# ROBOT-WSC/RGC-SLAM

Hardware: AMD Instinct MI355X
Metric: registered scans/sec (16-beam -> 1M-pt map) (higher is better)
Workload: dtype f32 points and neighbour search, f64 covariances and solve

## Files before the change

rgc-slam_amd/csrc/rgc_kernels.hip:

```cpp
#include "rgc_kernels.h"
#include "rgc_nn.h"
#include "rgc_lm.h"
#include "rgc_cov.h"
#include "rgc_terms.h"
#include <hip/hip_ext.h>

#include <limits.h>
#include <stddef.h>

#include <type_traits>

namespace rgck {

constexpr int WAVE = 64;

__device__ __forceinline__ int voxel_coord1(float x, double res) { return (int)floor((double)x / res - 0.5); }

__device__ __forceinline__ int wave_min(int v) {
#pragma unroll
  for (int o = 32; o > 0; o >>= 1) v = min(v, __shfl_xor(v, o));
  return v;
}
__device__ __forceinline__ int wave_max(int v) {
#pragma unroll
// ... 1504 lines not shown
    if (!kFinal) return true;
    defer(~i, (double)thr_up < 3.0 * (R + 1) * (R + 1) * g.res * g.res ? thr_up : INFINITY, 5);
    return false;
  }
  if (!decided) {
    defer(i, thr_up, 6);
    return false;
  }
  const int idx_k = swap ? index_of(a_k) : 0;
  const int m_lo = -(sub & 1), m_hi = -(sub >> 1);
  auto pick4 = [](int mlo, int mhi, int a0, int a1, int a2, int a3) {
    const int x = a0 ^ ((a0 ^ a1) & mlo), y = a2 ^ ((a2 ^ a3) & mlo);
    return x ^ ((x ^ y) & mhi);
  };
  int idx[KC];
  auto positions = [&](auto full_tag) {
    constexpr bool kFull = decltype(full_tag)::value;
#pragma unroll
    for (int t = 0; t < KC / S; t++) {
      const int key = pick4(m_lo, m_hi, all.a[S * t], all.a[S * t + 1], all.a[S * t + 2], all.a[S * t + 3]);
      const int j = S * t + sub;
      all.a[t] = (swap && j == k - 1) ? idx_k : ((kFull || j < k) ? index_of(key) : INT_MAX);
    }
    if (!df.split_sums) {
#pragma unroll
      for (int t = 0; t < KC / S; t++) {
        idx[S * t + 0] = quad_perm_i<0x00>(all.a[t]);
        idx[S * t + 1] = quad_perm_i<0x55>(all.a[t]);
        idx[S * t + 2] = quad_perm_i<0xAA>(all.a[t]);
        idx[S * t + 3] = quad_perm_i<0xFF>(all.a[t]);
      }
      sort_positions<KC>(idx);
      sp_normal_of<KC, kFull>(P, idx, px, py, pz, k, i, nx, ny, nz);
      return;
    }
    double S6[6] = {0, 0, 0, 0, 0, 0}, m3[3] = {0, 0, 0};
    const double qx = (double)px, qy = (double)py, qz = (double)pz;
#pragma unroll
    for (int t = 0; t < KC / S; t++) {
      const bool use = kFull || S * t + sub < k;
      const float4 cp = P[use ? all.a[t] : 0];
      const double dx = use ? (double)cp.x - qx : 0.0, dy = use ? (double)cp.y - qy : 0.0, dz = use ? (double)cp.z - qz : 0.0;
      m3[0] += dx; m3[1] += dy; m3[2] += dz;
      S6[0] = fma(dx, dx, S6[0]); S6[1] = fma(dx, dy, S6[1]); S6[2] = fma(dx, dz, S6[2]);
      S6[3] = fma(dy, dy, S6[3]); S6[4] = fma(dy, dz, S6[4]); S6[5] = fma(dz, dz, S6[5]);
    }
#pragma unroll
    for (int a = 0; a < 3; a++) m3[a] = quad_sum_f64(m3[a]);
#pragma unroll
    for (int a = 0; a < 6; a++) S6[a] = quad_sum_f64(S6[a]);
    normal_from_moments(S6, m3[0], m3[1], m3[2], k, i, nx, ny, nz);
  };
  if (kExact || k == KC) positions(std::true_type{});
  else positions(std::false_type{});
  return false;
}

template <bool kTarget> struct SpConfig {
  static constexpr int KB = kTarget ? 11 : 12;
  static constexpr int R = 1;
  static constexpr bool kClip = !kTarget;
  static constexpr int T = kTarget ? KNN_T : WAVE;
};

#if defined(RGC_LAB) || defined(RGC_LAB_BLK)
#define RGC_LAB_BLOCKS 1
__device__ long long g_lab_blk[4 * 16384];
void lab_blocks(long long* out) {
  (void)hipDeviceSynchronize();
  (void)hipMemcpyFromSymbol(out, HIP_SYMBOL(g_lab_blk), sizeof(g_lab_blk));
}
#endif
#ifdef RGC_LAB
__device__ long long g_lab_wave[2 * 8192];
void lab_wave_ts(long long* out, hipStream_t s) {
  (void)hipStreamSynchronize(s);
  (void)hipMemcpyFromSymbol(out, HIP_SYMBOL(g_lab_wave), sizeof(g_lab_wave));
}
#endif
constexpr int kSeedT = 128;
template <bool kTarget, bool kSeeded> struct SpLaunch : SpConfig<kTarget> {
  static constexpr int T = kSeeded ? kSeedT : SpConfig<kTarget>::T;
};
struct CoopRows {
  int pref[WAVE + 1];
  int rowa[WAVE];
  int nb[32];
};

template <int KC, int R, bool kExact>
__global__ void __launch_bounds__(WAVE)
k_knn_sp_wide(const float4* __restrict__ P, const int* __restrict__ start, Grid g, int n, int k, Deferred df, double* __restrict__ nx,
              double* __restrict__ ny, double* __restrict__ nz) {
  extern __shared__ int slist_wide[];
  if (df.guard && *df.guard) return;
  const int t = (int)blockIdx.x * WAVE + (int)threadIdx.x;
  const int i = t >> 2;
  if (i < n) knn_point_split<KC, SpConfig<false>::KB, R, WAVE, kExact>(P, start, g, n, k, i, t & 3, slist_wide + threadIdx.x, df, nx, ny, nz);
}

__device__ __forceinline__ int wave_sum_i(int v) {
#pragma unroll
  for (int o = 32; o > 0; o >>= 1) v += __shfl_xor(v, o);
  return v;
}
__device__ __forceinline__ int wave_min_i(int v) { return wave_min(v); }



__device__ __forceinline__ int coop_locate(const CoopRows* sh, int j) {
  int rr = 0;
#pragma unroll
  for (int step = 32; step > 0; step >>= 1) {
    const int probe = rr + step;
    if (sh->pref[probe] <= j) rr = probe;
  }
  return sh->rowa[rr] + (j - sh->pref[rr]);
}

template <typename F>
__device__ __forceinline__ void coop_for_each_candidate(const Grid& g, const int c[3], int r, const int* __restrict__ start,
                                                        CoopRows* sh, int lane, F&& f) {
  const int z0 = max(c[2] - r, 0), z1 = min(c[2] + r, g.dim[2] - 1);
  const int y0 = max(c[1] - r, 0), y1 = min(c[1] + r, g.dim[1] - 1);
  const int x0 = max(c[0] - r, 0), x1 = min(c[0] + r, g.dim[0] - 1);
  if (x0 > x1 || y0 > y1 || z0 > z1) return;
  const int ny = y1 - y0 + 1, nrows = ny * (z1 - z0 + 1);
  for (int rb = 0; rb < nrows; rb += WAVE) {
    const int t = rb + lane;
    int a = 0, b = 0;
    if (t < nrows) {
      const int y = y0 + t % ny, z = z0 + t / ny;
      a = start[cell_index(g, x0, y, z)];
      b = start[cell_index(g, x1, y, z) + 1];
    }
    const int len = b - a;
    int inc = len;
#pragma unroll
    for (int o = 1; o < WAVE; o <<= 1) {
      const int u = __shfl_up(inc, o);
      if (lane >= o) inc += u;
    }
    const int total = __shfl(inc, WAVE - 1);
    wave_lds_fence();
    sh->pref[lane] = inc - len;
    sh->rowa[lane] = a;
    if (lane == 0) sh->pref[WAVE] = INT_MAX;
    wave_lds_fence();
    for (int jb = 0; jb < total; jb += 2 * WAVE) {
      const int j0 = jb + lane, j1 = jb + WAVE + lane;
      const bool v0 = j0 < total, v1 = j1 < total;
      const int s0 = v0 ? coop_locate(sh, j0) : 0;
      const int s1 = v1 ? coop_locate(sh, j1) : 0;
      f(s0, v0, s1, v1);
    }
  }
}

template <int KW>
__device__ __forceinline__ unsigned coop_kth(const float4* __restrict__ P, const int* __restrict__ start, const Grid& g, const int c[3], int r,
                                             CoopRows* sh, int lane, float px, float py, float pz, int k, bool& overflow) {
  TopK<KW> top;
  top.init();
  coop_for_each_candidate(g, c, r, start, sh, lane, [&](int s0, bool v0, int s1, bool v1) {
    const float4 c0 = P[s0], c1 = P[s1];
    const float x0 = v0 ? dist2(px, py, pz, c0) : INFINITY;
    const float x1 = v1 ? dist2(px, py, pz, c1) : INFINITY;
    if (top.improves(x0)) top.insert(x0);
    if (top.improves(x1)) top.insert(x1);
  });
  unsigned T = 0;
  for (int bit = 30; bit >= 0; bit--) {
    const unsigned cand = T | (1u << bit);
    if (cand > 0x7F800000u) continue;
    int cnt_lt = 0;
#pragma unroll
    for (int j = 0; j < KW; j++) cnt_lt += __popcll(__ballot(top.a[j] < (int)cand));
    if (cnt_lt < k) T = cand;
  }
  overflow = __any(top.a[KW - 1] < (int)T);
  return T;
}

struct GenOut { double* c6; int method; int n; };
template <int KC>
__device__ __forceinline__ void cov6_of(const float4* __restrict__ P, const int (&idx)[KC], int k, int i, const GenOut& go);

template <int KC, bool kTarget, bool kGeneral = false, bool kLean = false>
__device__ __forceinline__ void coop_one(const float4* __restrict__ P, const int* __restrict__ start, const Grid& g, int k, const Deferred& df,
                                         double* __restrict__ nx, double* __restrict__ ny, double* __restrict__ nz, CoopRows* sh, int lane,
                                         int e, int enc, float thr, const GenOut& go = GenOut{nullptr, 0, 0}) {
  {
#ifdef RGC_LAB
    const long long lab_t0 = wall_clock64();
    int lab_rounds = 0;
#endif
    const int i = enc < 0 ? ~enc : enc;
    int r = enc < 0 ? 1 : 0;
    const float4 pq = P[i];
    const float px = pq.x, py = pq.y, pz = pq.z;
    const int c[3] = {cell_coord(px, g) - g.minc[0], cell_coord(py, g) - g.minc[1], cell_coord(pz, g) - g.minc[2]};
    const double q[3] = {(double)px, (double)py, (double)pz};
    const int rmax = max(max(max(c[0], g.dim[0] - 1 - c[0]), max(c[1], g.dim[1] - 1 - c[1])), max(c[2], g.dim[2] - 1 - c[2]));
    for (;;) {
      int rn;
      if (thr < INFINITY) {
        const double need = sqrt((double)thr) * (1.0 + 1e-5);
        rn = r + 1;
        while (rn < rmax) {
          const double b = cube_bound(g, c, q, rn);
          if (b == 1.0e300 || b > need) break;
          rn++;
        }
      } else {
        rn = r + max(1, (r + 1) / 2);
      }
      r = min(rn, rmax);
      bool overflow;
#ifdef RGC_LAB
      lab_rounds++;
#endif
      unsigned T = coop_kth<4>(P, start, g, c, r, sh, lane, px, py, pz, k, overflow);
      if (overflow) T = coop_kth<KC>(P, start, g, c, r, sh, lane, px, py, pz, k, overflow);
      thr = (T >= 0x7F800000u) ? INFINITY : __uint_as_float(T);
      if (r >= rmax) break;
      if (thr < INFINITY) {
        const double bound = cube_bound(g, c, q, r);
        if (bound == 1.0e300) break;
        if (bound > 0.0 && (double)thr < bound * bound * (1.0 - 1e-5)) break;
      }
    }
    int m = 0;
    int tie_o = INT_MAX, tie_s = -1;
    auto take = [&](int s, bool valid, const float4& cp) {
      const float x = valid ? dist2(px, py, pz, cp) : INFINITY;
      const unsigned long long mask = __ballot(x < thr);
      if (x < thr) {
        const int pos = m + __popcll(mask & ((1ull << lane) - 1ull));
        if (pos < k) sh->nb[pos] = s;
      }
      m += __popcll(mask);
      const int o = __float_as_int(cp.w);
      if (x == thr && o < tie_o) { tie_o = o; tie_s = s; }
    };
    coop_for_each_candidate(g, c, r, start, sh, lane, [&](int s0, bool v0, int s1, bool v1) {
      const float4 c0 = P[s0], c1 = P[s1];
      take(s0, v0, c0);
      take(s1, v1, c1);
    });
    int last_o = -1;
    while (m < k) {
      int best_o = wave_min_i(tie_o);
      if (best_o == INT_MAX) break;
      if (tie_o == best_o) sh->nb[m] = tie_s;
      m++;
      last_o = best_o;
      if (m >= k) break;
      tie_o = INT_MAX;
      tie_s = -1;
      coop_for_each_candidate(g, c, r, start, sh, lane, [&](int s0, bool v0, int s1, bool v1) {
        const float4 c0 = P[s0], c1 = P[s1];
        const int o0 = __float_as_int(c0.w), o1 = __float_as_int(c1.w);
        if (v0 && dist2(px, py, pz, c0) == thr && o0 > last_o && o0 < tie_o) { tie_o = o0; tie_s = s0; }
        if (v1 && dist2(px, py, pz, c1) == thr && o1 > last_o && o1 < tie_o) { tie_o = o1; tie_s = s1; }
      });
    }
    wave_lds_fence();
    {
      const int mine = lane < k ? sh->nb[lane] : INT_MAX;
      int rank = 0;
      for (int j = 0; j < k; j++) rank += sh->nb[j] < mine;
      wave_lds_fence();
      if (lane < k) sh->nb[rank] = mine;
      wave_lds_fence();
    }
    if constexpr (kLean) {
      static_assert(!kGeneral && KC <= 32, "coordinates of up to 32 neighbours in the rows' LDS");
      if (lane < k) {
        const float4 cp = P[sh->nb[lane]];
        sh->pref[lane] = __float_as_int(cp.x); sh->pref[32 + lane] = __float_as_int(cp.y); sh->rowa[lane] = __float_as_int(cp.z);
      }
      wave_lds_fence();
      if (lane == 0) {
        double S[6] = {0, 0, 0, 0, 0, 0};
        const double qx = (double)px, qy = (double)py, qz = (double)pz;
        double mx = 0, my = 0, mz = 0;
#pragma unroll 1
        for (int j = 0; j < k; j++) {
          const double dx = (double)__int_as_float(sh->pref[j]) - qx, dy = (double)__int_as_float(sh->pref[32 + j]) - qy, dz = (double)__int_as_float(sh->rowa[j]) - qz;
          mx += dx; my += dy; mz += dz;
          S[0] = fma(dx, dx, S[0]); S[1] = fma(dx, dy, S[1]); S[2] = fma(dx, dz, S[2]);
          S[3] = fma(dy, dy, S[3]); S[4] = fma(dy, dz, S[4]); S[5] = fma(dz, dz, S[5]);
        }
        normal_from_moments(S, mx, my, mz, k, i, nx, ny, nz);
        if (kTarget && df.seed) df.seed[__float_as_int(pq.w)] = thr;
      }
    } else if (lane == 0) {
      int idx[KC];
#pragma unroll
      for (int j = 0; j < KC; j++) idx[j] = j < k ? sh->nb[j] : 0;
      if constexpr (kGeneral) {
        cov6_of<KC>(P, idx, k, i, go);
      } else {
        if (k == KC) sp_normal_of<KC, true>(P, idx, px, py, pz, k, i, nx, ny, nz);
        else sp_normal_of<KC, false>(P, idx, px, py, pz, k, i, nx, ny, nz);
      }
      if (kTarget && df.seed) df.seed[__float_as_int(pq.w)] = thr;
#ifdef RGC_LAB
      if (!kTarget && e < 8192) { g_lab_wave[2 * e] = lab_t0 | ((long long)r << 56) | ((long long)lab_rounds << 48); g_lab_wave[2 * e + 1] = wall_clock64(); }
#endif
    }
    wave_lds_fence();
  }
}

template <int KC, bool kTarget>
__device__ __forceinline__ void coop_run(const float4* __restrict__ P, const int* __restrict__ start, const Grid& g, int k, const Deferred& df,
                                         double* __restrict__ nx, double* __restrict__ ny, double* __restrict__ nz, CoopRows* sh, int lane,
                                         int wave, int nwaves) {
  const int cnt = *df.cnt;
  for (int e = wave; e < cnt; e += nwaves) {
    const int enc = __builtin_amdgcn_readfirstlane(df.idx[e]);
    const float thr = __int_as_float(__builtin_amdgcn_readfirstlane(__float_as_int(df.thr[e])));
    coop_one<KC, kTarget>(P, start, g, k, df, nx, ny, nz, sh, lane, e, enc, thr);
  }
}
template <int KC, bool kTarget = false>
__device__ __forceinline__ void coop_stream(const float4* __restrict__ P, const int* __restrict__ start, const Grid& g, int k, const Deferred& df,
                            double* __restrict__ nx, double* __restrict__ ny, double* __restrict__ nz, CoopRows* sh, int lane, int wave, int nwaves,
                            int bulk_blocks, int nslots) {
  for (int e = wave;; e += nwaves) {
    if (e >= nslots) return;
    unsigned long long v;
    for (;;) {
      v = __hip_atomic_load(&df.slots[e], __ATOMIC_RELAXED, __HIP_MEMORY_SCOPE_AGENT);
      if (v != kSlotEmpty) break;
      __builtin_amdgcn_s_sleep(20);
    }
    if constexpr (kTarget) {
      const int enc0 = (int)(unsigned)v;
      const unsigned long long left = v == kSlotEnd ? kSlotEmpty : (kSlotResolvedTag | (unsigned long long)(unsigned)(enc0 < 0 ? ~enc0 : enc0));
      if (lane == 0) __hip_atomic_store(&df.slots[e], left, __ATOMIC_RELAXED, __HIP_MEMORY_SCOPE_AGENT);
    } else {
      if (lane == 0) __hip_atomic_store(&df.slots[e], kSlotEmpty, __ATOMIC_RELAXED, __HIP_MEMORY_SCOPE_AGENT);
    }
    if (v == kSlotEnd) return;
    const int enc = __builtin_amdgcn_readfirstlane((int)(unsigned)v);
    const float thr = __int_as_float(__builtin_amdgcn_readfirstlane((int)(unsigned)(v >> 32)));
    coop_one<KC, kTarget, false, kTarget>(P, start, g, k, df, nx, ny, nz, sh, lane, e, enc, thr);
  }
}
__device__ __forceinline__ void coop_count_out(const Deferred& df, int bulk_blocks, int nwaves, int nslots, int* flag) {
  __syncthreads();
  if (threadIdx.x == 0) *flag = __hip_atomic_fetch_add(df.done, 1, __ATOMIC_RELAXED, __HIP_MEMORY_SCOPE_AGENT) == bulk_blocks - 1;
  __syncthreads();
  if (*flag) {
    const int cnt = __hip_atomic_load(df.cnt, __ATOMIC_RELAXED, __HIP_MEMORY_SCOPE_AGENT);
    for (int j = (int)threadIdx.x; j < nwaves; j += (int)blockDim.x)
      if (cnt + j < nslots) __hip_atomic_store(&df.slots[cnt + j], kSlotEnd, __ATOMIC_RELAXED, __HIP_MEMORY_SCOPE_AGENT);
  }
}
struct VoxOut {
  double* vox;
  int* vox_cell;
  const int* cell_voxel;
};
__device__ __forceinline__ void voxel_block_from_search(const float4* __restrict__ P, const int* __restrict__ start, const Grid& g, int n, int i,
                                                        const double (&nrm)[3], const VoxOut& vo, int* lds);
template <int KC, bool kTarget>
__global__ void __launch_bounds__(WAVE)
k_knn_coop(const float4* __restrict__ P, const int* __restrict__ start, Grid g, int k, Deferred df, double* __restrict__ nx,
           double* __restrict__ ny, double* __restrict__ nz) {
  __shared__ CoopRows shm[1];
  wave_prio(!kTarget);
  if (df.guard && *df.guard) return;
  coop_run<KC, kTarget>(P, start, g, k, df, nx, ny, nz, &shm[0], (int)threadIdx.x, (int)blockIdx.x, (int)gridDim.x);
}

template <int KC, bool kTarget, bool kExact, bool kSeeded, bool kVox>
__device__ __forceinline__ void knn_sp_body(const float4* __restrict__ P, const int* __restrict__ start, const Grid& g, int n, int k, const Deferred& df,
                                            double* __restrict__ nx, double* __restrict__ ny, double* __restrict__ nz, const VoxOut& vo) {
  extern __shared__ __align__(16) int slist_sp[];
  using Cfg = SpLaunch<kTarget, kSeeded>;
  static_assert(!kSeeded || (kTarget && kExact), "seeds: the map's search at k == KC");
  wave_prio(!kTarget);
  if (df.guard && *df.guard) return;
  constexpr int kXcdRun = kXcdRunQueries / Cfg::T;
  int b = (int)blockIdx.x, slot = b >> 3;
  const int x = b & 7;
  if constexpr (!kTarget) {
    if (df.coop_blocks > 0 && b >= (int)gridDim.x - df.coop_blocks) {
      const int bulk = (int)gridDim.x - df.coop_blocks;
      coop_stream<KC>(P, start, g, k, df, nx, ny, nz, reinterpret_cast<CoopRows*>(slist_sp) + (threadIdx.x / WAVE), (int)threadIdx.x & (WAVE - 1),
                      (b - bulk) * (Cfg::T / WAVE) + (int)threadIdx.x / WAVE, df.coop_blocks * (Cfg::T / WAVE), bulk, n);
      return;
    }
    const int t = b * Cfg::T + (int)threadIdx.x;
    const int i = t >> 2;
#ifdef RGC_LAB
    const long long lab_t0 = wall_clock64();
#endif
    if (i < n && knn_point_split<KC, Cfg::KB, Cfg::R, Cfg::T, kExact, false>(P, start, g, n, k, i, t & 3, slist_sp + threadIdx.x, df, nx, ny, nz))
      knn_point_split<KC, Cfg::KB, 2, Cfg::T, kExact, true>(P, start, g, n, k, i, t & 3, slist_sp + threadIdx.x, df, nx, ny, nz);
#ifdef RGC_LAB
    if (threadIdx.x == 0 && b < 8192) { g_lab_wave[2 * b] = lab_t0; g_lab_wave[2 * b + 1] = wall_clock64(); }
#endif
    if (df.coop_blocks > 0) coop_count_out(df, (int)gridDim.x - df.coop_blocks, df.coop_blocks * (Cfg::T / WAVE), n, slist_sp);
    return;
  }
  if constexpr (kVox) {
    if (df.coop_blocks > 0 && b >= (int)gridDim.x - df.coop_blocks) {
      const int bulk = (int)gridDim.x - df.coop_blocks;
      coop_stream<KC, true>(P, start, g, k, df, nx, ny, nz, reinterpret_cast<CoopRows*>(slist_sp) + (threadIdx.x / WAVE), (int)threadIdx.x & (WAVE - 1),
                            (b - bulk) * (Cfg::T / WAVE) + (int)threadIdx.x / WAVE, df.coop_blocks * (Cfg::T / WAVE), bulk, n);
      return;
    }
  }
  bool cached = false;
  if constexpr (kSeeded && RGC_KNN_CACHE != 0) {
    if (df.cache.nbr) {
      const bool redo = cache_redo(df.cache);
      if (b < df.cache_nb) {
        if (redo) return;
        Deferred dfb = df;
        dfb.cache.nbr = nullptr;
        const int l = b % kTodoLists, per = df.cache_nb / kTodoLists;
        const int cnt = min(df.cache.todo_cnt[l], df.cache.todo_cap);
        for (int e = (b / kTodoLists) * Cfg::T + (int)threadIdx.x; e < cnt; e += per * Cfg::T) {
          const int q = df.cache.pos_of[df.cache.todo[(size_t)l * df.cache.todo_cap + e]];
          if (!knn_point_seeded<KC, Cfg::KB, Cfg::T>(P, start, g, n, q, slist_sp + threadIdx.x, dfb, nx, ny, nz))
            knn_point_sp<KC, Cfg::KB, Cfg::R, Cfg::T, kExact>(P, start, g, n, k, q, slist_sp + threadIdx.x, dfb, nx, ny, nz);
        }
// ... 164 lines not shown
    const int t0 = sh.head_t[h], cc = sh.head_c[h];
    const int vv = cell_voxel[cc];
    const bool last = h == H - 1;
    const int e_in = last ? bend - b0 : sh.head_t[h + 1];
    const int e1 = last ? start[cc + 1] : b0 + e_in;
    if (!kSpill && e1 > bend) continue;
    const double* __restrict__ row = sh.t[k];
    double acc = 0.0;
    for (int u = t0; u < e_in; u++) acc += row[u];
    if constexpr (kSpill)
      for (int u = b0 + e_in; u < e1; u++) acc += voxel_term(P, nx, ny, nz, k, u);
    const double num = (double)(e1 - (b0 + t0));
    vox[(size_t)vv * kVoxRec + k] = acc / num;
    if (k == 0) {
      vox[(size_t)vv * kVoxRec + 9] = num;
      vox_cell[vv] = cc;
    }
  }
}
__device__ __forceinline__ void voxel_build_block(const float4* __restrict__ P, const double* __restrict__ nx, const double* __restrict__ ny,
                                                  const double* __restrict__ nz, const int* __restrict__ start, const Grid& g, int n,
                                                  const int* __restrict__ cell_voxel, double* __restrict__ vox, int* __restrict__ vox_cell,
                                                  VoxLds& sh, int block) {
  const int b0 = block * VOX_T, bend = min(b0 + VOX_T, n);
  const int s = b0 + threadIdx.x;
  int c = 0;
  bool head = false;
  if (s < n) {
    const float4 cp = P[s], pv = P[s > 0 ? s - 1 : 0];
    const double a = nx[s], b = ny[s], d = nz[s];
    c = cell_index(g, cell_coord(cp.x, g) - g.minc[0], cell_coord(cp.y, g) - g.minc[1], cell_coord(cp.z, g) - g.minc[2]);
    const int cprev = cell_index(g, cell_coord(pv.x, g) - g.minc[0], cell_coord(pv.y, g) - g.minc[1], cell_coord(pv.z, g) - g.minc[2]);
    head = s == 0 || cprev != c;
    sh.t[0][threadIdx.x] = (double)cp.x;
    sh.t[1][threadIdx.x] = (double)cp.y;
    sh.t[2][threadIdx.x] = (double)cp.z;
    sh.t[3][threadIdx.x] = 1.0 - 0.999 * a * a;
    sh.t[4][threadIdx.x] = -0.999 * a * b;
    sh.t[5][threadIdx.x] = -0.999 * a * d;
    sh.t[6][threadIdx.x] = 1.0 - 0.999 * b * b;
    sh.t[7][threadIdx.x] = -0.999 * b * d;
    sh.t[8][threadIdx.x] = 1.0 - 0.999 * d * d;
  }
  voxel_block_sums<true>(P, nx, ny, nz, start, cell_voxel, vox, vox_cell, sh, b0, bend, c, head);
}
static_assert(KNN_T == VOX_T, "the search's workgroup is the voxel pass's block");
static_assert(sizeof(VoxLds) <= sizeof(int) * SpShape<SpConfig<true>::R, SpConfig<true>::kClip>::LDS * KNN_T, "VoxLds fits the search's LDS columns");
__device__ __forceinline__ void voxel_block_from_search(const float4* __restrict__ P, const int* __restrict__ start, const Grid& g, int n, int i,
                                                        const double (&nrm)[3], const VoxOut& vo, int* lds) {
  VoxLds& sh = *reinterpret_cast<VoxLds*>(lds);
  const int b0 = i - (int)threadIdx.x, bend = min(b0 + VOX_T, n);
  int c = 0;
  bool head = false;
  if (i < n) {
    const float4 cp = P[i], pv = P[i > 0 ? i - 1 : 0];
    const double a = nrm[0], b = nrm[1], d = nrm[2];
    c = cell_index(g, cell_coord(cp.x, g) - g.minc[0], cell_coord(cp.y, g) - g.minc[1], cell_coord(cp.z, g) - g.minc[2]);
    const int cprev = cell_index(g, cell_coord(pv.x, g) - g.minc[0], cell_coord(pv.y, g) - g.minc[1], cell_coord(pv.z, g) - g.minc[2]);
    head = i == 0 || cprev != c;
    sh.t[0][threadIdx.x] = (double)cp.x;
    sh.t[1][threadIdx.x] = (double)cp.y;
    sh.t[2][threadIdx.x] = (double)cp.z;
    sh.t[3][threadIdx.x] = 1.0 - 0.999 * a * a;
    sh.t[4][threadIdx.x] = -0.999 * a * b;
    sh.t[5][threadIdx.x] = -0.999 * a * d;
    sh.t[6][threadIdx.x] = 1.0 - 0.999 * b * b;
    sh.t[7][threadIdx.x] = -0.999 * b * d;
    sh.t[8][threadIdx.x] = 1.0 - 0.999 * d * d;
  }
  voxel_block_sums<false>(P, nullptr, nullptr, nullptr, start, vo.cell_voxel, vo.vox, vo.vox_cell, sh, b0, bend, c, head);
}
__global__ void __launch_bounds__(VOX_T)
k_voxel_build(const float4* __restrict__ P, const double* __restrict__ nx, const double* __restrict__ ny, const double* __restrict__ nz,
              const int* __restrict__ start, Grid g, int n, const int* __restrict__ cell_voxel, double* __restrict__ vox,
              int* __restrict__ vox_cell) {
  __shared__ VoxLds sh;
  voxel_build_block(P, nx, ny, nz, start, g, n, cell_voxel, vox, vox_cell, sh, (int)blockIdx.x);
}
template <int KC>
__global__ void __launch_bounds__(VOX_T, 1)
k_voxel_build_coop(const float4* __restrict__ P, double* __restrict__ nx, double* __restrict__ ny, double* __restrict__ nz,
                   const int* __restrict__ start, Grid g, int n, const int* __restrict__ cell_voxel, double* __restrict__ vox,
                   int* __restrict__ vox_cell, int nb_coop, int k, Deferred df) {
  __shared__ VoxLds sh;
  __shared__ CoopRows shm[VOX_T / WAVE];
  if (df.guard && *df.guard) return;
  if ((int)blockIdx.x >= nb_coop) {
    voxel_build_block(P, nx, ny, nz, start, g, n, cell_voxel, vox, vox_cell, sh, (int)blockIdx.x - nb_coop);
    return;
  }
  const int w = (int)threadIdx.x / WAVE;
  coop_run<KC, true>(P, start, g, k, df, nx, ny, nz, &shm[w], (int)threadIdx.x & (WAVE - 1), (int)blockIdx.x * (VOX_T / WAVE) + w,
                     nb_coop * (VOX_T / WAVE));
}

__device__ __forceinline__ void voxel_of_cell_wave(const float4* __restrict__ P, const double* __restrict__ nx, const double* __restrict__ ny,
                                                   const double* __restrict__ nz, const int* __restrict__ start, int c, const int* __restrict__ cell_voxel,
                                                   double* __restrict__ vox, int* __restrict__ vox_cell, double (*term)[WAVE], int lane) {
  const int s0 = start[c], s1 = start[c + 1];
  double m[3] = {0, 0, 0}, C[6] = {0, 0, 0, 0, 0, 0};
  for (int b0 = s0; b0 < s1; b0 += WAVE) {
    const int u = b0 + lane;
    if (u < s1) {
      const float4 p0 = P[u];
      const double a = nx[u], b = ny[u], d = nz[u];
      term[0][lane] = (double)p0.x; term[1][lane] = (double)p0.y; term[2][lane] = (double)p0.z;
      term[3][lane] = 1.0 - 0.999 * a * a; term[4][lane] = -0.999 * a * b; term[5][lane] = -0.999 * a * d;
      term[6][lane] = 1.0 - 0.999 * b * b; term[7][lane] = -0.999 * b * d; term[8][lane] = 1.0 - 0.999 * d * d;
    }
    wave_lds_fence();
    if (lane == 0) {
      const int nb = min(WAVE, s1 - b0);
      for (int t = 0; t < nb; t++) {
        m[0] += term[0][t]; m[1] += term[1][t]; m[2] += term[2][t];
        C[0] += term[3][t]; C[1] += term[4][t]; C[2] += term[5][t];
        C[3] += term[6][t]; C[4] += term[7][t]; C[5] += term[8][t];
      }
    }
    wave_lds_fence();
  }
  if (lane == 0) {
    const double num = (double)(s1 - s0);
    const int v = cell_voxel[c];
    if (vox_cell) vox_cell[v] = c;
    double* rec = vox + (size_t)v * kVoxRec;
    rec[0] = m[0] / num; rec[1] = m[1] / num; rec[2] = m[2] / num;
#pragma unroll
    for (int a = 0; a < 6; a++) rec[3 + a] = C[a] / num;
    rec[9] = num;
  }
}

__global__ void __launch_bounds__(WAVE)
k_voxel_patch(const float4* __restrict__ P, const double* __restrict__ nx, const double* __restrict__ ny, const double* __restrict__ nz,
              const int* __restrict__ start, Grid g, const int* __restrict__ deferred, const int* __restrict__ cell_voxel, double* __restrict__ vox) {
  __shared__ double term[9][WAVE];
  const int cnt = deferred[0];
  const int* idx = deferred + 16;
  const int lane = (int)threadIdx.x;
  for (int e = blockIdx.x; e < cnt; e += gridDim.x) {
    const int enc = idx[e];
    const int i = enc < 0 ? ~enc : enc;
    const float4 cp = P[i];
    const int c = cell_index(g, cell_coord(cp.x, g) - g.minc[0], cell_coord(cp.y, g) - g.minc[1], cell_coord(cp.z, g) - g.minc[2]);
    voxel_of_cell_wave(P, nx, ny, nz, start, c, cell_voxel, vox, nullptr, term, lane);
  }
}

__global__ void __launch_bounds__(WAVE)
k_voxel_seams(const float4* __restrict__ P, const double* __restrict__ nx, const double* __restrict__ ny, const double* __restrict__ nz,
              const int* __restrict__ start, Grid g, int n, int* __restrict__ deferred, const int* __restrict__ cell_voxel, double* __restrict__ vox,
              int* __restrict__ vox_cell, int nseam, const int* __restrict__ guard) {
  __shared__ double term[9][WAVE];
  if (guard && *guard) return;
  const int lane = (int)threadIdx.x;
  if ((int)blockIdx.x < nseam) {
    const int s = ((int)blockIdx.x + 1) * VOX_T;
    if (s >= n) return;
    const float4 cp = P[s], pv = P[s - 1];
    const int c = cell_index(g, cell_coord(cp.x, g) - g.minc[0], cell_coord(cp.y, g) - g.minc[1], cell_coord(cp.z, g) - g.minc[2]);
    const int cprev = cell_index(g, cell_coord(pv.x, g) - g.minc[0], cell_coord(pv.y, g) - g.minc[1], cell_coord(pv.z, g) - g.minc[2]);
    if (c != cprev || start[c] < s - VOX_T) return;
    voxel_of_cell_wave(P, nx, ny, nz, start, c, cell_voxel, vox, vox_cell, term, lane);
    return;
  }
  const int cnt = deferred[0];
  unsigned long long* slots = reinterpret_cast<unsigned long long*>(deferred + 16);
  for (int e = (int)blockIdx.x - nseam; e < cnt; e += (int)gridDim.x - nseam) {
    const int i = __builtin_amdgcn_readfirstlane((int)(unsigned)slots[e]);
    if (lane == 0) slots[e] = kSlotEmpty;
    if ((unsigned)i >= (unsigned)n) continue;
    const float4 cp = P[i];
    const int c = cell_index(g, cell_coord(cp.x, g) - g.minc[0], cell_coord(cp.y, g) - g.minc[1], cell_coord(cp.z, g) - g.minc[2]);
    voxel_of_cell_wave(P, nx, ny, nz, start, c, cell_voxel, vox, vox_cell, term, lane);
  }
}

template <int KC>
__global__ void __launch_bounds__(VOX_T)
k_voxel_cells_coop(const float4* __restrict__ P, double* __restrict__ nx, double* __restrict__ ny, double* __restrict__ nz,
                   const int* __restrict__ start, Grid g, const int* __restrict__ cell_voxel, double* __restrict__ vox, int* __restrict__ vox_cell,
                   int nb_coop, int k, Deferred df, const int* __restrict__ cell_list, const int* __restrict__ ncells) {
  __shared__ double term[VOX_T / WAVE][9][WAVE];
  __shared__ CoopRows shm[VOX_T / WAVE];
  const int w = (int)threadIdx.x / WAVE, lane = (int)threadIdx.x & (WAVE - 1);
  if ((int)blockIdx.x < nb_coop) {
    if (df.guard && *df.guard) return;
    coop_run<KC, true>(P, start, g, k, df, nx, ny, nz, &shm[w], lane, (int)blockIdx.x * (VOX_T / WAVE) + w, nb_coop * (VOX_T / WAVE));
    return;
  }
  if (df.guard && *df.guard) return;
  const int nc = *ncells, nwaves = ((int)gridDim.x - nb_coop) * (VOX_T / WAVE);
  for (int e = ((int)blockIdx.x - nb_coop) * (VOX_T / WAVE) + w; e < nc; e += nwaves) {
    const float4 cp = P[cell_list[e]];
    const int c = cell_index(g, cell_coord(cp.x, g) - g.minc[0], cell_coord(cp.y, g) - g.minc[1], cell_coord(cp.z, g) - g.minc[2]);
    voxel_of_cell_wave(P, nx, ny, nz, start, c, cell_voxel, vox, vox_cell, term[w], lane);
  }
}

constexpr int LIN_T = 256;
int linearize_blocks(int n) { return (n + LIN_T - 1) / LIN_T; }

__device__ __forceinline__ void neighbor_offset(int noff, int o, int& ox, int& oy, int& oz) {
  if (noff == 1) { ox = oy = oz = 0; return; }
  if (noff == 7) {
    ox = (o == 1) - (o == 2);
    oy = (o == 3) - (o == 4);
    oz = (o == 5) - (o == 6);
    return;
  }
  ox = o / 9 - 1; oy = (o / 3) % 3 - 1; oz = o % 3 - 1;
}

template <int NACC, bool kWriteThrough = false>
__device__ __forceinline__ void block_reduce_store(double (&acc)[NACC], double* __restrict__ row) {
  static_assert(NACC <= 32 && LIN_T == 256, "thread -> (accumulator, eighth) mapping");
  if constexpr (NACC <= 2) {
    static_assert(!kWriteThrough, "no row of one or two sums is handed over inside a launch");
    block_sum_store<LIN_T>(acc, row);
  } else {
    constexpr int PITCH = NACC | 1;
    __shared__ double quads[LIN_T / 4][PITCH];
    __shared__ double eighths[8][32];
    const int q = threadIdx.x >> 2;
#pragma unroll
    for (int a = 0; a < NACC; a++) {
      double v = acc[a];
      v += quad_perm_f64<0xB1>(v);
      v += quad_perm_f64<0x4E>(v);
      if ((threadIdx.x & 3) == 0) quads[q][a] = v;
    }
    __syncthreads();
    const int a = threadIdx.x & 31, e = threadIdx.x >> 5;
    if (a < NACC) {
      double t = quads[e * 8][a];
#pragma unroll
      for (int j = 1; j < 8; j++) t += quads[e * 8 + j][a];
      eighths[e][a] = t;
    }
    __syncthreads();
    if (threadIdx.x < NACC) {
      double t = eighths[0][threadIdx.x];
#pragma unroll
      for (int j = 1; j < 8; j++) t += eighths[j][threadIdx.x];
      if (kWriteThrough) __hip_atomic_store(&row[threadIdx.x], t, __ATOMIC_RELAXED, __HIP_MEMORY_SCOPE_AGENT);
      else row[threadIdx.x] = t;
    }
  }
}

__device__ __forceinline__ void rcrt6_of_normal(const Pose& T, const double a0, const double a1, const double a2, double (&CA)[6]) {
  const double r0 = T.R[0] * a0 + T.R[1] * a1 + T.R[2] * a2;
  const double r1 = T.R[3] * a0 + T.R[4] * a1 + T.R[5] * a2;
  const double r2 = T.R[6] * a0 + T.R[7] * a1 + T.R[8] * a2;
  CA[0] = 1.0 - 0.999 * r0 * r0; CA[1] = -0.999 * r0 * r1; CA[2] = -0.999 * r0 * r2;
  CA[3] = 1.0 - 0.999 * r1 * r1; CA[4] = -0.999 * r1 * r2; CA[5] = 1.0 - 0.999 * r2 * r2;
}

__device__ __forceinline__ void linearize_point(const float4 pp, const double (&CA)[6], int i, int n, const Pose& T, const Grid& g,
                                                const int* __restrict__ cell_voxel, const double* __restrict__ vox, int noff,
                                                int* __restrict__ corr_v, double* __restrict__ corr_M, int want_H, double (&acc)[kAccum],
                                                int& ncorr, int* __restrict__ miss = nullptr, const int* __restrict__ need = nullptr, int stamp = 0) {
    const double p0 = (double)pp.x, p1 = (double)pp.y, p2 = (double)pp.z;
    const double q0 = T.R[0] * p0 + T.R[1] * p1 + T.R[2] * p2 + T.t[0];
    const double q1 = T.R[3] * p0 + T.R[4] * p1 + T.R[5] * p2 + T.t[1];
    const double q2 = T.R[6] * p0 + T.R[7] * p1 + T.R[8] * p2 + T.t[2];
    const int cx = (int)floor(q0 / g.res - 0.5) - g.minc[0];
// ... 1367 lines not shown
```

Measured before the change: 2908.

## Cache cooperative kNN candidates in LDS and parallelise normal and voxel moment sums

The cooperative kNN path now stores up to 256 candidate indices, distances and coordinates in per-wave LDS during the first top-k pass. When everything fits, the final neighbour selection and tie-breaking read from LDS instead of rescanning the grid and reloading points. Normal moments are now accumulated with one of nine lanes per moment term rather than serially on lane 0, and the voxel moment reduction is split the same way. LDS for the coop and voxel/build roles is unioned to offset the larger CoopRows, though the bigger per-wave footprint may still reduce occupancy.

```diff
diff --git a/rgc-slam_amd/csrc/rgc_kernels.hip b/rgc-slam_amd/csrc/rgc_kernels.hip
--- a/rgc-slam_amd/csrc/rgc_kernels.hip
+++ b/rgc-slam_amd/csrc/rgc_kernels.hip
@@ -1610,10 +1610,16 @@
 template <bool kTarget, bool kSeeded> struct SpLaunch : SpConfig<kTarget> {
   static constexpr int T = kSeeded ? kSeedT : SpConfig<kTarget>::T;
 };
+constexpr int kCoopCap = 4 * WAVE;
 struct CoopRows {
   int pref[WAVE + 1];
   int rowa[WAVE];
   int nb[32];
+  int nbo[32];
+  float nbx[3][32];
+  int cpos[kCoopCap];
+  float cd[kCoopCap];
+  float cxyz[3][kCoopCap];
 };
 
 template <int KC, int R, bool kExact>
@@ -1647,13 +1653,14 @@
 }
 
 template <typename F>
-__device__ __forceinline__ void coop_for_each_candidate(const Grid& g, const int c[3], int r, const int* __restrict__ start,
-                                                        CoopRows* sh, int lane, F&& f) {
+__device__ __forceinline__ int coop_for_each_candidate(const Grid& g, const int c[3], int r, const int* __restrict__ start,
+                                                       CoopRows* sh, int lane, F&& f) {
   const int z0 = max(c[2] - r, 0), z1 = min(c[2] + r, g.dim[2] - 1);
   const int y0 = max(c[1] - r, 0), y1 = min(c[1] + r, g.dim[1] - 1);
   const int x0 = max(c[0] - r, 0), x1 = min(c[0] + r, g.dim[0] - 1);
-  if (x0 > x1 || y0 > y1 || z0 > z1) return;
+  if (x0 > x1 || y0 > y1 || z0 > z1) return 0;
   const int ny = y1 - y0 + 1, nrows = ny * (z1 - z0 + 1);
+  int base = 0;
   for (int rb = 0; rb < nrows; rb += WAVE) {
     const int t = rb + lane;
     int a = 0, b = 0;
@@ -1680,32 +1687,43 @@
       const bool v0 = j0 < total, v1 = j1 < total;
       const int s0 = v0 ? coop_locate(sh, j0) : 0;
       const int s1 = v1 ? coop_locate(sh, j1) : 0;
-      f(s0, v0, s1, v1);
-    }
-  }
+      f(base + j0, s0, v0, base + j1, s1, v1);
+    }
+    base += total;
+  }
+  return base;
 }
 
 template <int KW>
-__device__ __forceinline__ unsigned coop_kth(const float4* __restrict__ P, const int* __restrict__ start, const Grid& g, const int c[3], int r,
-                                             CoopRows* sh, int lane, float px, float py, float pz, int k, bool& overflow) {
-  TopK<KW> top;
-  top.init();
-  coop_for_each_candidate(g, c, r, start, sh, lane, [&](int s0, bool v0, int s1, bool v1) {
-    const float4 c0 = P[s0], c1 = P[s1];
-    const float x0 = v0 ? dist2(px, py, pz, c0) : INFINITY;
-    const float x1 = v1 ? dist2(px, py, pz, c1) : INFINITY;
-    if (top.improves(x0)) top.insert(x0);
-    if (top.improves(x1)) top.insert(x1);
-  });
+__device__ __forceinline__ unsigned coop_bisect(const int (&a)[KW], int k) {
   unsigned T = 0;
   for (int bit = 30; bit >= 0; bit--) {
     const unsigned cand = T | (1u << bit);
     if (cand > 0x7F800000u) continue;
     int cnt_lt = 0;
 #pragma unroll
-    for (int j = 0; j < KW; j++) cnt_lt += __popcll(__ballot(top.a[j] < (int)cand));
+    for (int j = 0; j < KW; j++) cnt_lt += __popcll(__ballot(a[j] < (int)cand));
     if (cnt_lt < k) T = cand;
   }
+  return T;
+}
+template <int KW, bool kCache>
+__device__ __forceinline__ unsigned coop_kth(const float4* __restrict__ P, const int* __restrict__ start, const Grid& g, const int c[3], int r,
+                                             CoopRows* sh, int lane, float px, float py, float pz, int k, bool& overflow, int& ncand) {
+  TopK<KW> top;
+  top.init();
+  ncand = coop_for_each_candidate(g, c, r, start, sh, lane, [&](int o0, int s0, bool v0, int o1, int s1, bool v1) {
+    const float4 c0 = P[s0], c1 = P[s1];
+    const float x0 = v0 ? dist2(px, py, pz, c0) : INFINITY;
+    const float x1 = v1 ? dist2(px, py, pz, c1) : INFINITY;
+    if constexpr (kCache) {
+      if (v0 && o0 < kCoopCap) { sh->cpos[o0] = s0; sh->cd[o0] = x0; sh->cxyz[0][o0] = c0.x; sh->cxyz[1][o0] = c0.y; sh->cxyz[2][o0] = c0.z; }
+      if (v1 && o1 < kCoopCap) { sh->cpos[o1] = s1; sh->cd[o1] = x1; sh->cxyz[0][o1] = c1.x; sh->cxyz[1][o1] = c1.y; sh->cxyz[2][o1] = c1.z; }
+    }
+    if (top.improves(x0)) top.insert(x0);
+    if (top.improves(x1)) top.insert(x1);
+  });
+  const unsigned T = coop_bisect<KW>(top.a, k);
   overflow = __any(top.a[KW - 1] < (int)T);
   return T;
 }
@@ -1714,7 +1732,7 @@
 template <int KC>
 __device__ __forceinline__ void cov6_of(const float4* __restrict__ P, const int (&idx)[KC], int k, int i, const GenOut& go);
 
-template <int KC, bool kTarget, bool kGeneral = false, bool kLean = false>
+template <int KC, bool kTarget, bool kGeneral = false>
 __device__ __forceinline__ void coop_one(const float4* __restrict__ P, const int* __restrict__ start, const Grid& g, int k, const Deferred& df,
                                          double* __restrict__ nx, double* __restrict__ ny, double* __restrict__ nz, CoopRows* sh, int lane,
                                          int e, int enc, float thr, const GenOut& go = GenOut{nullptr, 0, 0}) {
@@ -1730,6 +1748,7 @@
     const int c[3] = {cell_coord(px, g) - g.minc[0], cell_coord(py, g) - g.minc[1], cell_coord(pz, g) - g.minc[2]};
     const double q[3] = {(double)px, (double)py, (double)pz};
     const int rmax = max(max(max(c[0], g.dim[0] - 1 - c[0]), max(c[1], g.dim[1] - 1 - c[1])), max(c[2], g.dim[2] - 1 - c[2]));
+    int ncand = 0;
     for (;;) {
       int rn;
       if (thr < INFINITY) {
@@ -1748,8 +1767,8 @@
 #ifdef RGC_LAB
       lab_rounds++;
 #endif
-      unsigned T = coop_kth<4>(P, start, g, c, r, sh, lane, px, py, pz, k, overflow);
-      if (overflow) T = coop_kth<KC>(P, start, g, c, r, sh, lane, px, py, pz, k, overflow);
+      unsigned T = coop_kth<4, true>(P, start, g, c, r, sh, lane, px, py, pz, k, overflow, ncand);
+      if (overflow) T = coop_kth<KC, false>(P, start, g, c, r, sh, lane, px, py, pz, k, overflow, ncand);
       thr = (T >= 0x7F800000u) ? INFINITY : __uint_as_float(T);
       if (r >= rmax) break;
       if (thr < INFINITY) {
@@ -1759,84 +1778,147 @@
       }
     }
     int m = 0;
-    int tie_o = INT_MAX, tie_s = -1;
-    auto take = [&](int s, bool valid, const float4& cp) {
-      const float x = valid ? dist2(px, py, pz, cp) : INFINITY;
-      const unsigned long long mask = __ballot(x < thr);
-      if (x < thr) {
-        const int pos = m + __popcll(mask & ((1ull << lane) - 1ull));
-        if (pos < k) sh->nb[pos] = s;
+    const bool cached = ncand <= kCoopCap && thr < INFINITY;
+    if (cached) {
+      constexpr int NT = kCoopCap / WAVE;
+      const unsigned long long below = (1ull << lane) - 1ull;
+      wave_lds_fence();
+      int cs[NT];
+      float cx[NT];
+#pragma unroll
+      for (int t = 0; t < NT; t++) {
+        const int o = lane + t * WAVE;
+        cs[t] = o < ncand ? sh->cpos[o] : 0;
+        cx[t] = o < ncand ? sh->cd[o] : INFINITY;
       }
-      m += __popcll(mask);
-      const int o = __float_as_int(cp.w);
-      if (x == thr && o < tie_o) { tie_o = o; tie_s = s; }
-    };
-    coop_for_each_candidate(g, c, r, start, sh, lane, [&](int s0, bool v0, int s1, bool v1) {
-      const float4 c0 = P[s0], c1 = P[s1];
-      take(s0, v0, c0);
-      take(s1, v1, c1);
-    });
-    int last_o = -1;
-    while (m < k) {
-      int best_o = wave_min_i(tie_o);
-      if (best_o == INT_MAX) break;
-      if (tie_o == best_o) sh->nb[m] = tie_s;
-      m++;
-      last_o = best_o;
-      if (m >= k) break;
-      tie_o = INT_MAX;
-      tie_s = -1;
-      coop_for_each_candidate(g, c, r, start, sh, lane, [&](int s0, bool v0, int s1, bool v1) {
+      int nties = 0;
+#pragma unroll
+      for (int t = 0; t < NT; t++) {
+        const unsigned long long mask = __ballot(cx[t] < thr);
+        if (cx[t] < thr) {
+          const int pos = m + __popcll(mask & below);
+          if (pos < k) { sh->nb[pos] = cs[t]; sh->nbo[pos] = lane + t * WAVE; }
+        }
+        m += __popcll(mask);
+        nties += __popcll(__ballot(cx[t] == thr));
+      }
+      if (m + nties <= k) {
+#pragma unroll
+        for (int t = 0; t < NT; t++) {
+          const unsigned long long mask = __ballot(cx[t] == thr);
+          if (cx[t] == thr) {
+            const int pos = m + __popcll(mask & below);
+            if (pos < k) { sh->nb[pos] = cs[t]; sh->nbo[pos] = lane + t * WAVE; }
+          }
+          m += __popcll(mask);
+        }
+      } else {
+        int co[NT];
+#pragma unroll
+        for (int t = 0; t < NT; t++) co[t] = cx[t] == thr ? __float_as_int(P[cs[t]].w) : INT_MAX;
+        int last_o = -1;
+        while (m < k) {
+          int bo = INT_MAX, bs = -1, bq = 0;
+#pragma unroll
+          for (int t = 0; t < NT; t++)
+            if (co[t] > last_o && co[t] < bo) { bo = co[t]; bs = cs[t]; bq = lane + t * WAVE; }
+          const int best_o = wave_min_i(bo);
+          if (best_o == INT_MAX) break;
+          if (bo == best_o) { sh->nb[m] = bs; sh->nbo[m] = bq; }
+          m++;
+          last_o = best_o;
+        }
+      }
+    } else {
+      int tie_o = INT_MAX, tie_s = -1;
+      auto take = [&](int s, bool valid, const float4& cp) {
+        const float x = valid ? dist2(px, py, pz, cp) : INFINITY;
+        const unsigned long long mask = __ballot(x < thr);
+        if (x < thr) {
+          const int pos = m + __popcll(mask & ((1ull << lane) - 1ull));
+          if (pos < k) sh->nb[pos] = s;
+        }
+        m += __popcll(mask);
+        const int o = __float_as_int(cp.w);
+        if (x == thr && o < tie_o) { tie_o = o; tie_s = s; }
+      };
+      coop_for_each_candidate(g, c, r, start, sh, lane, [&](int, int s0, bool v0, int, int s1, bool v1) {
         const float4 c0 = P[s0], c1 = P[s1];
-        const int o0 = __float_as_int(c0.w), o1 = __float_as_int(c1.w);
-        if (v0 && dist2(px, py, pz, c0) == thr && o0 > last_o && o0 < tie_o) { tie_o = o0; tie_s = s0; }
-        if (v1 && dist2(px, py, pz, c1) == thr && o1 > last_o && o1 < tie_o) { tie_o = o1; tie_s = s1; }
+        take(s0, v0, c0);
+        take(s1, v1, c1);
       });
+      int last_o = -1;
+      while (m < k) {
+        int best_o = wave_min_i(tie_o);
+        if (best_o == INT_MAX) break;
+        if (tie_o == best_o) sh->nb[m] = tie_s;
+        m++;
+        last_o = best_o;
+        if (m >= k) break;
+        tie_o = INT_MAX;
+        tie_s = -1;
+        coop_for_each_candidate(g, c, r, start, sh, lane, [&](int, int s0, bool v0, int, int s1, bool v1) {
+          const float4 c0 = P[s0], c1 = P[s1];
+          const int o0 = __float_as_int(c0.w), o1 = __float_as_int(c1.w);
+          if (v0 && dist2(px, py, pz, c0) == thr && o0 > last_o && o0 < tie_o) { tie_o = o0; tie_s = s0; }
+          if (v1 && dist2(px, py, pz, c1) == thr && o1 > last_o && o1 < tie_o) { tie_o = o1; tie_s = s1; }
+        });
+      }
     }
     wave_lds_fence();
     {
       const int mine = lane < k ? sh->nb[lane] : INT_MAX;
+      float mc[3] = {0.0f, 0.0f, 0.0f};
+      if constexpr (!kGeneral) {
+        if (lane < k) {
+          if (cached) {
+            const int o = sh->nbo[lane];
+            mc[0] = sh->cxyz[0][o]; mc[1] = sh->cxyz[1][o]; mc[2] = sh->cxyz[2][o];
+          } else {
+            const float4 cp = P[mine];
+            mc[0] = cp.x; mc[1] = cp.y; mc[2] = cp.z;
+          }
+        }
+      }
       int rank = 0;
       for (int j = 0; j < k; j++) rank += sh->nb[j] < mine;
       wave_lds_fence();
-      if (lane < k) sh->nb[rank] = mine;
-      wave_lds_fence();
-    }
-    if constexpr (kLean) {
-      static_assert(!kGeneral && KC <= 32, "coordinates of up to 32 neighbours in the rows' LDS");
       if (lane < k) {
-        const float4 cp = P[sh->nb[lane]];
-        sh->pref[lane] = __float_as_int(cp.x); sh->pref[32 + lane] = __float_as_int(cp.y); sh->rowa[lane] = __float_as_int(cp.z);
+        sh->nb[rank] = mine;
+        if constexpr (!kGeneral) { sh->nbx[0][rank] = mc[0]; sh->nbx[1][rank] = mc[1]; sh->nbx[2][rank] = mc[2]; }
       }
       wave_lds_fence();
+    }
+    if constexpr (!kGeneral) {
+      static_assert(KC <= 32, "coordinates of up to 32 neighbours in the wave's LDS");
+      const int a = lane < 9 ? lane : 0;
+      const int ua = a < 3 ? a : (a < 6 ? 0 : (a < 8 ? 1 : 2));
+      const int va = a < 3 ? 0 : (a < 6 ? a - 3 : (a < 8 ? a - 5 : 2));
+      const double qu = (double)(ua == 0 ? px : (ua == 1 ? py : pz)), qv = (double)(va == 0 ? px : (va == 1 ? py : pz));
+      double acc = 0;
+#pragma unroll 4
+      for (int j = 0; j < k; j++) {
+        const double du = (double)sh->nbx[ua][j] - qu;
+        const double dv = a < 3 ? 1.0 : (double)sh->nbx[va][j] - qv;
+        acc = fma(du, dv, acc);
+      }
+      double S[6];
+      const double mx = __shfl(acc, 0), my = __shfl(acc, 1), mz = __shfl(acc, 2);
+#pragma unroll
+      for (int j = 0; j < 6; j++) S[j] = __shfl(acc, 3 + j);
       if (lane == 0) {
-        double S[6] = {0, 0, 0, 0, 0, 0};
-        const double qx = (double)px, qy = (double)py, qz = (double)pz;
-        double mx = 0, my = 0, mz = 0;
-#pragma unroll 1
-        for (int j = 0; j < k; j++) {
-          const double dx = (double)__int_as_float(sh->pref[j]) - qx, dy = (double)__int_as_float(sh->pref[32 + j]) - qy, dz = (double)__int_as_float(sh->rowa[j]) - qz;
-          mx += dx; my += dy; mz += dz;
-          S[0] = fma(dx, dx, S[0]); S[1] = fma(dx, dy, S[1]); S[2] = fma(dx, dz, S[2]);
-          S[3] = fma(dy, dy, S[3]); S[4] = fma(dy, dz, S[4]); S[5] = fma(dz, dz, S[5]);
-        }
         normal_from_moments(S, mx, my, mz, k, i, nx, ny, nz);
         if (kTarget && df.seed) df.seed[__float_as_int(pq.w)] = thr;
+#ifdef RGC_LAB
+        const int slot = kTarget ? 8191 - e : e;
+        if (slot >= 0 && slot < 8192) { g_lab_wave[2 * slot] = lab_t0 | ((long long)r << 56) | ((long long)lab_rounds << 48); g_lab_wave[2 * slot + 1] = wall_clock64(); }
+#endif
       }
     } else if (lane == 0) {
       int idx[KC];
 #pragma unroll
       for (int j = 0; j < KC; j++) idx[j] = j < k ? sh->nb[j] : 0;
-      if constexpr (kGeneral) {
-        cov6_of<KC>(P, idx, k, i, go);
-      } else {
-        if (k == KC) sp_normal_of<KC, true>(P, idx, px, py, pz, k, i, nx, ny, nz);
-        else sp_normal_of<KC, false>(P, idx, px, py, pz, k, i, nx, ny, nz);
-      }
-      if (kTarget && df.seed) df.seed[__float_as_int(pq.w)] = thr;
-#ifdef RGC_LAB
-      if (!kTarget && e < 8192) { g_lab_wave[2 * e] = lab_t0 | ((long long)r << 56) | ((long long)lab_rounds << 48); g_lab_wave[2 * e + 1] = wall_clock64(); }
-#endif
+      cov6_of<KC>(P, idx, k, i, go);
     }
     wave_lds_fence();
   }
@@ -1875,7 +1957,7 @@
     if (v == kSlotEnd) return;
     const int enc = __builtin_amdgcn_readfirstlane((int)(unsigned)v);
     const float thr = __int_as_float(__builtin_amdgcn_readfirstlane((int)(unsigned)(v >> 32)));
-    coop_one<KC, kTarget, false, kTarget>(P, start, g, k, df, nx, ny, nz, sh, lane, e, enc, thr);
+    coop_one<KC, kTarget>(P, start, g, k, df, nx, ny, nz, sh, lane, e, enc, thr);
   }
 }
 __device__ __forceinline__ void coop_count_out(const Deferred& df, int bulk_blocks, int nwaves, int nslots, int* flag) {
@@ -2206,13 +2288,14 @@
 k_voxel_build_coop(const float4* __restrict__ P, double* __restrict__ nx, double* __restrict__ ny, double* __restrict__ nz,
                    const int* __restrict__ start, Grid g, int n, const int* __restrict__ cell_voxel, double* __restrict__ vox,
                    int* __restrict__ vox_cell, int nb_coop, int k, Deferred df) {
-  __shared__ VoxLds sh;
-  __shared__ CoopRows shm[VOX_T / WAVE];
+  constexpr size_t kLds = sizeof(VoxLds) > sizeof(CoopRows) * (VOX_T / WAVE) ? sizeof(VoxLds) : sizeof(CoopRows) * (VOX_T / WAVE);
+  __shared__ __align__(16) unsigned char lds[kLds];
   if (df.guard && *df.guard) return;
   if ((int)blockIdx.x >= nb_coop) {
-    voxel_build_block(P, nx, ny, nz, start, g, n, cell_voxel, vox, vox_cell, sh, (int)blockIdx.x - nb_coop);
+    voxel_build_block(P, nx, ny, nz, start, g, n, cell_voxel, vox, vox_cell, *reinterpret_cast<VoxLds*>(lds), (int)blockIdx.x - nb_coop);
     return;
   }
+  CoopRows* shm = reinterpret_cast<CoopRows*>(lds);
   const int w = (int)threadIdx.x / WAVE;
   coop_run<KC, true>(P, start, g, k, df, nx, ny, nz, &shm[w], (int)threadIdx.x & (WAVE - 1), (int)blockIdx.x * (VOX_T / WAVE) + w,
                      nb_coop * (VOX_T / WAVE));
@@ -2222,7 +2305,9 @@
                                                    const double* __restrict__ nz, const int* __restrict__ start, int c, const int* __restrict__ cell_voxel,
                                                    double* __restrict__ vox, int* __restrict__ vox_cell, double (*term)[WAVE], int lane) {
   const int s0 = start[c], s1 = start[c + 1];
-  double m[3] = {0, 0, 0}, C[6] = {0, 0, 0, 0, 0, 0};
+  const int v = cell_voxel[c];
+  double acc = 0;
+  const int row = lane < 9 ? lane : 0;
   for (int b0 = s0; b0 < s1; b0 += WAVE) {
     const int u = b0 + lane;
     if (u < s1) {
@@ -2233,24 +2318,16 @@
       term[6][lane] = 1.0 - 0.999 * b * b; term[7][lane] = -0.999 * b * d; term[8][lane] = 1.0 - 0.999 * d * d;
     }
     wave_lds_fence();
-    if (lane == 0) {
-      const int nb = min(WAVE, s1 - b0);
-      for (int t = 0; t < nb; t++) {
-        m[0] += term[0][t]; m[1] += term[1][t]; m[2] += term[2][t];
-        C[0] += term[3][t]; C[1] += term[4][t]; C[2] += term[5][t];
-        C[3] += term[6][t]; C[4] += term[7][t]; C[5] += term[8][t];
-      }
-    }
+    const int nb = min(WAVE, s1 - b0);
+#pragma unroll 4
+    for (int t = 0; t < nb; t++) acc += term[row][t];
     wave_lds_fence();
   }
+  const double num = (double)(s1 - s0);
+  double* rec = vox + (size_t)v * kVoxRec;
+  if (lane < 9) rec[lane] = acc / num;
   if (lane == 0) {
-    const double num = (double)(s1 - s0);
-    const int v = cell_voxel[c];
     if (vox_cell) vox_cell[v] = c;
-    double* rec = vox + (size_t)v * kVoxRec;
-    rec[0] = m[0] / num; rec[1] = m[1] / num; rec[2] = m[2] / num;
-#pragma unroll
-    for (int a = 0; a < 6; a++) rec[3 + a] = C[a] / num;
     rec[9] = num;
   }
 }
@@ -2305,8 +2382,11 @@
 k_voxel_cells_coop(const float4* __restrict__ P, double* __restrict__ nx, double* __restrict__ ny, double* __restrict__ nz,
                    const int* __restrict__ start, Grid g, const int* __restrict__ cell_voxel, double* __restrict__ vox, int* __restrict__ vox_cell,
                    int nb_coop, int k, Deferred df, const int* __restrict__ cell_list, const int* __restrict__ ncells) {
-  __shared__ double term[VOX_T / WAVE][9][WAVE];
-  __shared__ CoopRows shm[VOX_T / WAVE];
+  using Terms = double[VOX_T / WAVE][9][WAVE];
+  constexpr size_t kLds = sizeof(Terms) > sizeof(CoopRows) * (VOX_T / WAVE) ? sizeof(Terms) : sizeof(CoopRows) * (VOX_T / WAVE);
+  __shared__ __align__(16) unsigned char lds[kLds];
+  Terms& term = *reinterpret_cast<Terms*>(lds);
+  CoopRows* shm = reinterpret_cast<CoopRows*>(lds);
   const int w = (int)threadIdx.x / WAVE, lane = (int)threadIdx.x & (WAVE - 1);
   if ((int)blockIdx.x < nb_coop) {
     if (df.guard && *df.guard) return;
```

After: 2915, median of 6. About the same (+0.2%).
